# airl-iisc/MRFP

Hardware: AMD Instinct MI355X
Metric: train images/sec (higher is better)
Workload: dtype bf16; 1 GPU; resnet-101 DeepLabV3+ + MRFP+ (HRFP+NP+ on, HRFP re-drawn every step), 768x768, 16 images/GPU, fwd+bwd+SGD, synthetic 19-class, random-init weights; global_batch=16, parallelism=dp1

## Files before the change

### include/mrfp_hip.h

```cpp
#ifndef MRFP_HIP_H
#define MRFP_HIP_H

#include <stdint.h>

#ifdef __cplusplus
extern "C" {
#endif

typedef enum { MRFP_F32 = 0, MRFP_BF16 = 1, MRFP_F16 = 2 } mrfp_dtype;

int mrfp_version(void);
const char* mrfp_last_error(void);

int64_t mrfp_stats_nslab(int64_t B, int64_t Ho);

int mrfp_stats_fwd(const void* x, int dtype, int64_t B, int64_t Ho, int64_t Wo, int64_t C,
                   int64_t Hs, int64_t Ws, const int32_t* tabH, const int32_t* tabW,
                   float* ws, void* stream);

int mrfp_stats_bwd(const void* dy, const void* x, const void* y, const float* mean,
                   const float* fA, const float* fS, int per_image, int dtype, int64_t B, int64_t Ho, int64_t Wo, int64_t C,
                   int64_t Hs, int64_t Ws, const int32_t* tabH, const int32_t* tabW,
                   float* ws, void* stream);
int mrfp_stats_bwd_mask(const void* dy, const void* x, const void* mask, const float* mean, int per_image, int dtype, int64_t B,
// ... 138 lines not shown
                  int64_t sstride, const void* addend, float* colstats, void* stream);
int mrfp_conv_fwd_act(const void* x, const void* wpack, const float* bias, void* y, int dtype,
                      int64_t B, int64_t H, int64_t W, int64_t C, int64_t N, int64_t ldy, int64_t R, int64_t S,
                      int64_t Ho, int64_t Wo, int64_t stride, int64_t pad_h, int64_t pad_w, int64_t dil,
                      int64_t sstride, const void* addend, int act, void* stream);
int mrfp_pack_weight_folded(const float* w, void* wf, const float* conv_bias, const float* bn_weight, const float* bn_bias,
                            const float* running_mean, const float* running_var, float eps, float* bias_out, int dtype,
                            int64_t N, int64_t C, int64_t R, int64_t S, int64_t Npad, int64_t Cpad, void* stream);
int mrfp_pack_weights_folded_batched(const void* jobs, const int64_t* prefix, int64_t njobs, int64_t total, int dtype, void* stream);
int mrfp_conv_stats_layout(int dtype, int64_t B, int64_t H, int64_t W, int64_t C, int64_t N, int64_t ldy, int64_t R, int64_t S,
                           int64_t Ho, int64_t Wo, int64_t stride, int64_t pad_h, int64_t pad_w, int64_t dil, int64_t sstride, int wstats,
                           int64_t* out);
int64_t mrfp_conv_stats_block_rows(int dtype, int64_t B, int64_t H, int64_t W, int64_t C, int64_t N, int64_t R, int64_t S, int64_t Ho,
                                   int64_t Wo, int64_t stride, int64_t pad_h, int64_t pad_w, int64_t dil, int64_t sstride);
int mrfp_conv_single_launch(int64_t B, int64_t image_bytes);
int mrfp_conv_fwd_wstats(const void* x, const void* wpack, const float* bias, void* y, int dtype,
                         int64_t B, int64_t H, int64_t W, int64_t C, int64_t N, int64_t ldy, int64_t R, int64_t S,
                         int64_t Ho, int64_t Wo, int64_t stride, int64_t pad_h, int64_t pad_w, int64_t dil,
                         const uint8_t* rowweight, float* colstats, void* stream);
int mrfp_conv_fwd_gated(const void* x, const void* wpack, const float* bias, void* y, int dtype,
                        int64_t B, int64_t H, int64_t W, int64_t C, int64_t N, int64_t ldy, int64_t R, int64_t S,
                        int64_t Ho, int64_t Wo, int64_t stride, int64_t pad_h, int64_t pad_w, int64_t dil,
                        int64_t sstride, const void* addend, const void* addend_mask, void* stream);
int mrfp_debug_clock_stamps(int family, uint64_t* out, int64_t n);
int64_t mrfp_conv_wgrad_ws_bytes(int64_t M, int64_t N, int64_t Q);
int mrfp_conv_wgrad(const void* x, const void* dy, float* dw, void* ws, int dtype,
                    int64_t B, int64_t H, int64_t W, int64_t C, int64_t Ctrue, int64_t N, int64_t ldn,
                    int64_t R, int64_t S, int64_t Ho, int64_t Wo, int64_t stride, int64_t pad_h, int64_t pad_w,
                    int64_t dil, void* stream);
int64_t mrfp_conv_wgrad_group_max(void);
int64_t mrfp_conv_wgrad_grouped_ws_bytes(int64_t M, int64_t N, int64_t Q, int64_t count);
int mrfp_conv_wgrad_plan(int dtype, int64_t B, int64_t H, int64_t W, int64_t C, int64_t N, int64_t ldn, int64_t R, int64_t S, int64_t Ho,
                         int64_t Wo, int64_t stride, int64_t pad_h, int64_t pad_w, int64_t dil, int64_t count, int64_t* out);
int mrfp_conv_wgrad_grouped(const void* const* xs, const void* const* dys, float* const* dws, int64_t count, void* ws, int dtype,
                            int64_t B, int64_t H, int64_t W, int64_t C, int64_t Ctrue, int64_t N, int64_t ldn,
                            int64_t R, int64_t S, int64_t Ho, int64_t Wo, int64_t stride, int64_t pad_h, int64_t pad_w,
                            int64_t dil, void* stream);
int mrfp_nchw_to_nhwc_pad(const float* x, void* y, int dtype, int64_t B, int64_t C, int64_t H, int64_t W,
                          int64_t Cpad, void* stream);

int mrfp_sgd_step(float* p, const float* g, float* m, int64_t n, float lr, float momentum,
                  float weight_decay, float gscale, int first, void* stream);

int64_t mrfp_grad_check_nblocks(int64_t n);
int mrfp_grad_check(const float* g, int64_t n, float gscale, void* ws, void* state, int dynamic, float growth,
                    float backoff, int growth_interval, float max_norm, void* stream);
// ... 76 lines not shown
```

### mrfp_amd/conv.py

```python
from __future__ import annotations

import collections
import ctypes
import os as _os
import warnings
import weakref
from typing import Any, NamedTuple, Optional

import torch

from . import _lib
from ._lib import call, dt, ptr, stream
from .ops import CL, GRAD_DEFERRED, _chk, channel_sums, empty_cl, grad_sink, notify_grad, wgrad_workspace, zeros_cl
from .ops import _inside_autograd_engine as _in_backward

_PACKS = {}
FUSE_STATS = [_os.environ.get("MRFP_FUSE_STATS", "1") != "0"]


class ConvStats(NamedTuple):
    final: torch.Tensor
    final_count: int
    elements: int
    rows: torch.Tensor
# ... 518 lines not shown
    return t


def _boundary_hook(_grad):
    flush_wgrads()
    return None


GATED_SKIP_HITS = [0]


def ungate(t):
    g = getattr(t, "_mrfp_gate", None) if t is not None else None
    if g is None:
        return t
    if g[1] != t._version:
        raise _lib.MrfpHipError("a gated skip gradient was modified in place before it reached its consumer")
    B, C, H, W = t.shape
    out = empty_cl(B, C, H, W, t.dtype, t.device)
    call("mrfp_affine_bwd_mask", ptr(t), None, ptr(g[0]), ptr(out), None, dt(t), B, H, W, C, None, None, None, 0, stream())
    return out


def L_single(B, H, W, Cphys, Ho, Wo, Nphys, esz):
    return max(B * H * W * Cphys, B * Ho * Wo * Nphys) * esz < 0xF0000000


class _Conv2d(torch.autograd.Function):

    @staticmethod
    def forward(ctx, x, weight, bias, stride, pad_h, pad_w, dil, Nphys, want_skip, stats, wtab):
        B, Cphys, H, W = x.shape
        N, C, R, S = weight.shape
        Ho, Wo = _out_size(H, R, stride, pad_h, dil), _out_size(W, S, stride, pad_w, dil)
        pk = get_pack(weight, bias, x.dtype, Cphys, Nphys)
        y = empty_cl(B, Nphys, Ho, Wo, x.dtype, x.device)
        _lib.NOTE[0] = (C, N)
        if wtab is not None:
            call("mrfp_conv_fwd_wstats", ptr(x), ptr(pk.wf), ptr(pk.bias), ptr(y), dt(x), B, H, W, Cphys, Nphys, Nphys, R, S,
                 Ho, Wo, stride, pad_h, pad_w, dil, ptr(wtab), ptr(stats), stream())
            WSTATS_HITS[0] += 1
        else:
            call("mrfp_conv_fwd", ptr(x), ptr(pk.wf), ptr(pk.bias), ptr(y), dt(x), B, H, W, Cphys, Nphys, Nphys, R, S,
                 Ho, Wo, stride, pad_h, pad_w, dil, 1, None, ptr(stats), stream())
        ctx.save_for_backward(x, weight, bias)
        ctx.cfg = (stride, pad_h, pad_w, dil, Nphys, Ho, Wo)
        ctx.set_materialize_grads(False)
        if want_skip:
            return y, x.view_as(x)
        return y

    @staticmethod
    def backward(ctx, dy, dskip=None):
        x, weight, bias = ctx.saved_tensors
        cell = getattr(ctx, "_mrfp_cell", None)
        if cell is not None and cell[1]:
            g = getattr(dskip, "_mrfp_gate", None) if dskip is not None else None
            if g is None or g[1] != dskip._version:
                raise _lib.MrfpHipError("a gated skip gradient reached its convolution without its gate: the skip alias was "
                                        "also consumed by an operator outside mrfp_amd.ops (set MRFP_GATED_SKIP=0)")
            cell[1] = False
        if dy is None:
            return (ungate(dskip),) + (None,) * 10
        stride, pad_h, pad_w, dil, Nphys, Ho, Wo = ctx.cfg
        dy = _chk(dy, "dy")
        B, Cphys, H, W = x.shape
        N, C, R, S = weight.shape
        dx = dw = db = None
        if ctx.needs_input_grad[0]:
            pk = get_pack(weight, bias, x.dtype, Cphys, Nphys)
            dx = empty_cl(B, Cphys, H, W, x.dtype, x.device)
            gate = None
            if dskip is not None:
                g = getattr(dskip, "_mrfp_gate", None)
                if g is not None:
                    if (g[1] == dskip._version and dskip.dtype == x.dtype and x.element_size() == 2
                            and Cphys % 8 == 0 and dskip.shape == dx.shape and dskip.is_contiguous(memory_format=CL)):
                        gate = g[0]
                    else:
                        dskip = ungate(dskip)
                dskip = _chk(dskip, "dskip")
                if dskip.dtype != x.dtype:
                    dskip = dskip.to(x.dtype)
            _lib.NOTE[0] = (N, C)
            if gate is not None:
                call("mrfp_conv_fwd_gated", ptr(dy), ptr(pk.wd), None, ptr(dx), dt(dy), B, Ho, Wo, Nphys, Cphys, Cphys, R, S, H, W,
                     1, dil * (R - 1) - pad_h, dil * (S - 1) - pad_w, dil, stride, ptr(dskip), ptr(gate), stream())
                GATED_SKIP_HITS[0] += 1
            else:
                call("mrfp_conv_fwd", ptr(dy), ptr(pk.wd), None, ptr(dx), dt(dy), B, Ho, Wo, Nphys, Cphys, Cphys, R, S, H, W,
                     1, dil * (R - 1) - pad_h, dil * (S - 1) - pad_w, dil, stride, ptr(dskip), None, stream())
        if ctx.needs_input_grad[1]:
            sig = (x.dtype, B, H, W, Cphys, C, N, Nphys, R, S, Ho, Wo, stride, pad_h, pad_w, dil)
            sink = grad_sink(weight)
            side = _WGRADS.stream(x.device) if sink is not None else None
            if sink is not None and GROUP_WGRAD[0] and L_single(B, H, W, Cphys, Ho, Wo, Nphys, x.element_size()):
                _WGRADS.submit(sig, x, dy, sink, weight)
            elif side is not None:
                _WGRADS.ensure_callback()
                _launch_wgrads(sig, [(x, dy, sink)], side)
                notify_grad(weight)
            else:
                dw = sink if sink is not None else torch.empty((N, C, R, S), dtype=torch.float32, device=x.device)
                _launch_wgrads(sig, [(x, dy, dw)], None)
                if sink is not None:
                    notify_grad(weight)
                    dw = None
                elif dw.dtype != weight.dtype:
                    dw = dw.to(weight.dtype)
        if bias is not None and ctx.needs_input_grad[2]:
            db = channel_sums(dy, N).to(bias.dtype)
        return (dx, dw, db) + (None,) * 8


class _SharedConv1x1Pair(torch.autograd.Function):

    @staticmethod
    def forward(ctx, x1, x2, weight, bias, Nphys):
        N, C, R, S = weight.shape
        if R != 1 or S != 1 or x1.shape[1] != C or x2.shape[1] != C:
            raise _lib.MrfpHipError("shared conv pair: 1x1 weight and unpadded inputs expected")
        pk = get_pack(weight, bias, x1.dtype, C, Nphys)
        ys = []
        for x, b in ((x1, None), (x2, pk.bias)):
            B, _, H, W = x.shape
            y = empty_cl(B, Nphys, H, W, x.dtype, x.device)
            call("mrfp_conv_fwd", ptr(x), ptr(pk.wf), ptr(b), ptr(y), dt(x), B, H, W, C, Nphys, Nphys, 1, 1, H, W, 1, 0, 0, 1, 1,
                 None, None, stream())
            ys.append(y)
        ctx.save_for_backward(x1, x2, weight, bias)
        ctx.Nphys = Nphys
        ctx.set_materialize_grads(False)
        return ys[0], ys[1]

    @staticmethod
    def backward(ctx, dy1, dy2):
        x1, x2, weight, bias = ctx.saved_tensors
        N, C, _, _ = weight.shape
        Nphys = ctx.Nphys
        pk = get_pack(weight, bias, x1.dtype, C, Nphys)
        dxs, dws = [], []
        db = None
        for x, dy, need_dx in ((x1, dy1, ctx.needs_input_grad[0]), (x2, dy2, ctx.needs_input_grad[1])):
            if dy is None:
                dxs.append(None)
                continue
            dy = _chk(dy, "dy")
            B, _, H, W = x.shape
            dx = None
            if need_dx:
                dx = empty_cl(B, C, H, W, x.dtype, x.device)
                call("mrfp_conv_fwd", ptr(dy), ptr(pk.wd), None, ptr(dx), dt(dy), B, H, W, Nphys, C, C, 1, 1, H, W, 1, 0, 0, 1, 1,
                     None, None, stream())
            dxs.append(dx)
            if ctx.needs_input_grad[2]:
                dw = torch.empty((N, C, 1, 1), dtype=torch.float32, device=x.device)
                _launch_wgrads((x.dtype, B, H, W, C, C, N, Nphys, 1, 1, H, W, 1, 0, 0, 1), [(x, dy, dw)], None)
                dws.append(dw)
        if bias is not None and ctx.needs_input_grad[3] and dy2 is not None:
            db = channel_sums(_chk(dy2, "dy"), N).to(bias.dtype)
        dw = None
        if dws:
            total = dws[0] if len(dws) == 1 else dws[0].add_(dws[1])
            sink = grad_sink(weight)
            if sink is not None:
                sink.copy_(total)
                notify_grad(weight)
            else:
                dw = total.to(weight.dtype)
        return dxs[0], dxs[1], dw, db, None


def shared_conv1x1_pair(x1, x2, weight, bias, phys_out):
# ... 31 lines not shown
                                "path is dense only" % (tuple(weight.shape), x.shape[1], groups))
    Nphys = phys_out if phys_out is not None else _round_up(N, epc)
    B, Cphys, H, W = x.shape
    R, S = weight.shape[2], weight.shape[3]
    Ho, Wo = _out_size(H, R, st, ph, dl), _out_size(W, S, st, pw, dl)
    L = _lib.lib()
    single = bool(L.mrfp_conv_single_launch(B, H * W * Cphys * x.element_size()))
    plan, wtab, stats = stat_resize, None, None
    if plan is not None and WSTATS[0] and FUSE_STATS[0] and single and (plan.Hs, plan.Ws) == (Ho, Wo) and R * S > 1:
        wtab = plan.multiplicity(B)
    if wtab is not None or (bias is None and FUSE_STATS[0] and single):
        lay = (ctypes.c_int64 * 5)()
        rc = L.mrfp_conv_stats_layout(dt(x), B, H, W, Cphys, Nphys, Nphys, R, S, Ho, Wo, st, ph, pw, dl, 1, int(wtab is not None), lay)
        if rc != 0:
            raise _lib.MrfpHipError("mrfp_conv_stats_layout failed (%d): %s" % (rc, L.mrfp_last_error().decode()))
        nblk, rb, rows, first, cnt = lay
        stats = torch.empty(rows * 2 * Nphys, dtype=torch.float32, device=x.device)
    if _WGRADS.callback_queued and not _in_backward():
        _WGRADS.drop_stale()
    out = _Conv2d.apply(x, weight, bias, st, ph, pw, dl, Nphys, want_skip, stats, wtab)
    y, skip = out if want_skip else (out, None)
    if skip is not None:
        skip._mrfp_skip_alias = True
        skip._mrfp_uses = [0, False]
        if y.grad_fn is not None:
            y.grad_fn._mrfp_cell = skip._mrfp_uses
    if stats is not None and (phys_out is not None or Nphys == N):
        final = stats[first * 2 * Nphys:(first + cnt) * 2 * Nphys]
        if wtab is not None:
            y._mrfp_colstats = ConvStats(final, cnt, B * plan.Ho * plan.Wo, stats, nblk, 0, plan, y._version)
        else:
            y._mrfp_colstats = ConvStats(final, cnt, B * Ho * Wo, stats, nblk, rb, None, y._version)
    if phys_out is None and Nphys != N:
        y = y[:, :N].contiguous(memory_format=CL)
    return (y, skip) if want_skip else y
```

### mrfp_amd/csrc/conv_c64.hip

```cpp
#include "conv_common.hpp"

namespace mrfp {


struct C64P {
    const char* x;
    const char* w;
    char* y;
    const float* bias;
    const char* addend;
    float* colstats;
    const unsigned char* rowweight;
    int B, H, W, N, ldy, dil;
    int strips;
    int units;
    int spi;
    unsigned xbytes, wbytes, ybytes;
};

constexpr int kC64Slots = 4;

template <typename T, int CB, int NCG, bool STATS, bool ADD, int ACT = 0>
__global__ __launch_bounds__(256, (CB == 1 ? 2 : 1)) void conv3x3_c64_kernel(C64P p) {
    constexpr int PSN = 4 / NCG;
    constexpr int SW = 64 * PSN;
    constexpr int NPIECE = (SW + 4 + 7) / 8;
    constexpr int NPC = CB * NPIECE;
    constexpr int PWV = (NPC + 3) / 4;
    constexpr int SLOT = NPC * 1024;
    constexpr int KS = 18 * CB;
    constexpr int PIXB = 128 * CB;
    constexpr int ST = 4;
    extern __shared__ __attribute__((aligned(16))) char smem[];
    const int t = threadIdx.x, lane = t & 63;
    const int wave = __builtin_amdgcn_readfirstlane(t >> 6);
    const int l15 = lane & 15, lq = lane >> 4;
    const int cg = wave % NCG, ps = wave / NCG;
    const int n0 = (int)blockIdx.y * 128 + cg * 32, nl = n0 + 8 * lq;
    const int d = p.dil;
    const unsigned lds0 = (unsigned)(size_t)(__attribute__((address_space(3))) char*)smem;
    const i32x4 xw = rsrc_words(p.x, p.xbytes);
    const __amdgpu_buffer_rsrc_t wr = __builtin_amdgcn_make_buffer_rsrc((void*)p.w, 0, (int)p.wbytes, 0x00020000);
    const __amdgpu_buffer_rsrc_t yr = __builtin_amdgcn_make_buffer_rsrc((void*)p.y, 0, (int)p.ybytes, 0x00020000);
    const __amdgpu_buffer_rsrc_t ar = __builtin_amdgcn_make_buffer_rsrc((void*)(p.addend ? p.addend : p.y), 0, (int)p.ybytes, 0x00020000);

    uint4 fw[KS][2];
#pragma unroll
    for (int ks = 0; ks < KS; ++ks)
#pragma unroll
        for (int j = 0; j < 2; ++j) {
            const int n = n0 + 8 * (l15 >> 2) + 4 * j + (l15 & 3);
            fw[ks][j] = bload(wr, n < p.N ? (unsigned)n * (unsigned)(1152 * CB) + (unsigned)(ks * 64 + lq * 16) : kOOB);
        }
#pragma unroll
    for (int ks = 0; ks < KS; ++ks)
#pragma unroll
        for (int j = 0; j < 2; ++j) settle(fw[ks][j]);
    float bv[2][4];
#pragma unroll
    for (int j = 0; j < 2; ++j)
#pragma unroll
        for (int e = 0; e < 4; ++e) bv[j][e] = (p.bias && nl + 4 * j + e < p.N) ? p.bias[nl + 4 * j + e] : 0.f;

    unsigned foff[3][2];
#pragma unroll
    for (int s = 0; s < 3; ++s) {
        const int px = ps * 64 + l15 + s * d;
#pragma unroll
        for (int kk = 0; kk < 2; ++kk) foff[s][kk] = (unsigned)(px * 128 + ((((kk * 4 + lq) ^ px) & 7) << 4));
    }

    float cs[8], cq[8];
#pragma unroll
    for (int u = 0; u < 8; ++u) { cs[u] = 0.f; cq[u] = 0.f; }

    const long long G = gridDim.x;
    int u = (int)((long long)blockIdx.x * p.units / G);
    const int u1 = (int)((long long)(blockIdx.x + 1) * p.units / G);
    const int Hc0 = (p.H + d - 1) / d;
    const int upi = p.strips * p.H;
// ... 62 lines not shown
                const unsigned cb = (unsigned)(col * PIXB + hf * 128 + (((lane & 7) ^ (px & 7)) << 4));
                dma16_async(xw, sbase + (unsigned)(pi * 1024), (rok && cok) ? rbase + cb : kOOB);
            }
        };
        issue_row(i0 - 1);
        issue_row(i0);
        issue_row(i0 + 1);
        for (int i = i0; i < i1; ++i) {
            if (i == i0) dma_wait<0>();
            else dma_wait<ST>();
            __builtin_amdgcn_s_barrier();
            if (i + 1 < i1) issue_row(i + 2);
            const int oh = q + d * i;
            uint4 av[4];
            unsigned wt[4];
            const int owl = ow0 + ps * 64 + l15;
            const unsigned ml = (unsigned)((b * p.H + oh) * p.W + owl);
            auto out_off = [&](int bk) {
                return (owl + bk * 16 < p.W && nl < p.N) ? ((ml + (unsigned)(bk * 16)) * (unsigned)p.ldy + (unsigned)nl) * 2u : kOOB;
            };
#pragma unroll
            for (int bk = 0; bk < 4; ++bk) {
                if constexpr (ADD) av[bk] = bload(ar, out_off(bk));
                if constexpr (STATS) {
                    const bool ok = owl + bk * 16 < p.W;
                    wt[bk] = ok ? (p.rowweight ? (unsigned)p.rowweight[ml + bk * 16] : 1u) : 0u;
                }
            }
            f32x4 acc[4][2];
            const unsigned sb[3] = {lds0 + (unsigned)(((i + 3) & 3) * SLOT), lds0 + (unsigned)((i & 3) * SLOT),
                                    lds0 + (unsigned)(((i + 1) & 3) * SLOT)};
            uint4 fx[2][4];
            auto read_x = [&](int ks, uint4 (&f)[4]) {
                const int r = ks / (6 * CB), s = (ks / (2 * CB)) % 3, hf = (ks >> 1) % CB, kk = ks & 1;
                const char* base = smem + (sb[r] - lds0) + hf * (NPIECE * 1024) + foff[s][kk];
#pragma unroll
                for (int bk = 0; bk < 4; ++bk) f[bk] = *reinterpret_cast<const uint4*>(base + bk * 2048);
            };
            read_x(0, fx[0]);
#pragma unroll
            for (int ks = 0; ks < KS; ++ks) {
                if (ks + 1 < KS) read_x(ks + 1, fx[(ks + 1) & 1]);
                __builtin_amdgcn_sched_barrier(0);
#pragma unroll
                for (int bk = 0; bk < 4; ++bk)
#pragma unroll
                    for (int j = 0; j < 2; ++j) {
                        if (ks == 0) {
                            const f32x4 z = {bv[j][0], bv[j][1], bv[j][2], bv[j][3]};
                            acc[bk][j] = z;
                        }
                        Mma16<T>::run(acc[bk][j], fw[ks][j], fx[ks & 1][bk]);
                    }
                __builtin_amdgcn_sched_barrier(0);
            }
#pragma unroll
            for (int bk = 0; bk < 4; ++bk) {
                uint4 v;
                if constexpr (ADD) {
                    float a[8];
                    unpack2<T>(av[bk].x, a[0], a[1]);
                    unpack2<T>(av[bk].y, a[2], a[3]);
                    unpack2<T>(av[bk].z, a[4], a[5]);
                    unpack2<T>(av[bk].w, a[6], a[7]);
                    v.x = pack2<T>(act_f<ACT>(acc[bk][0][0] + a[0]), act_f<ACT>(acc[bk][0][1] + a[1]));
                    v.y = pack2<T>(act_f<ACT>(acc[bk][0][2] + a[2]), act_f<ACT>(acc[bk][0][3] + a[3]));
                    v.z = pack2<T>(act_f<ACT>(acc[bk][1][0] + a[4]), act_f<ACT>(acc[bk][1][1] + a[5]));
                    v.w = pack2<T>(act_f<ACT>(acc[bk][1][2] + a[6]), act_f<ACT>(acc[bk][1][3] + a[7]));
                } else {
                    v.x = pack2<T>(act_f<ACT>(acc[bk][0][0]), act_f<ACT>(acc[bk][0][1]));
                    v.y = pack2<T>(act_f<ACT>(acc[bk][0][2]), act_f<ACT>(acc[bk][0][3]));
                    v.z = pack2<T>(act_f<ACT>(acc[bk][1][0]), act_f<ACT>(acc[bk][1][1]));
                    v.w = pack2<T>(act_f<ACT>(acc[bk][1][2]), act_f<ACT>(acc[bk][1][3]));
                }
                if constexpr (STATS) {
                    float f[8];
                    unpack2<T>(v.x, f[0], f[1]);
                    unpack2<T>(v.y, f[2], f[3]);
                    unpack2<T>(v.z, f[4], f[5]);
                    unpack2<T>(v.w, f[6], f[7]);
                    const float wb = (float)wt[bk];
#pragma unroll
// ... 29 lines not shown
        if (!c128 || (p.N != 64 && p.N != 128 && p.N != 256)) return false;
        const int SW = p.N == 64 ? 128 : 64;
        if (c128 < 2 && (int64_t)p.B * ((p.W + SW - 1) / SW) * p.H < 32 * kGrid1PerCU) return false;
    } else return false;
    if (p.addend_mask || (p.colstats && p.addend)) return false;
    if ((int64_t)p.M * p.ldy * esz >= (int64_t)kOOB || p.H < 2 * p.dil) return false;
    return true;
}
bool c64_plan(const ConvP& p, int esz, ConvPlan& plan) {
    if (!c64_applicable(p, esz)) return false;
    const int SW = p.N == 64 ? 128 : 64;
    const int64_t upi = (int64_t)((p.W + SW - 1) / SW) * p.H, units = upi * p.B;
    const int64_t cap = p.C == 64 ? kGrid2PerCU : kGrid1PerCU;
    plan.kind = ConvKernel::c64;
    plan.tile_rows = 0;
    plan.grid = (int)(units < cap ? units : cap);
    plan.spi = (int)(upi / (units / plan.grid) + 2);
    const int64_t rows_per_image = (int64_t)(p.N == 64 ? 2 : 1) * plan.spi;
    plan.stats_blocks = p.B * rows_per_image;
    plan.stats_block_rows = -rows_per_image;
    return true;
}

template <typename T, int CB, int NCG, bool STATS, bool ADD, int ACT = 0>
static int c64_launch(const C64P& q, int grid, hipStream_t st) {
    constexpr int SW = 64 * (4 / NCG), NPIECE = (SW + 4 + 7) / 8;
    const int lds = kC64Slots * CB * NPIECE * 1024 + 1024;
    static bool attr_set = false;
    if (!attr_set) {
        (void)hipFuncSetAttribute(reinterpret_cast<const void*>(&conv3x3_c64_kernel<T, CB, NCG, STATS, ADD, ACT>),
                                  hipFuncAttributeMaxDynamicSharedMemorySize, lds);
        attr_set = true;
    }
    hipLaunchKernelGGL((conv3x3_c64_kernel<T, CB, NCG, STATS, ADD, ACT>), dim3((unsigned)grid, (unsigned)((q.N + 127) / 128)), dim3(256), lds, st, q);
    MRFP_LAUNCH_CHECK();
    return 0;
}
template <typename T, int CB, int NCG>
static int c64_pick(const ConvP& p, const C64P& q, int grid, hipStream_t st, int act) {
    if (act != 0) {
        if (p.colstats) return -1;
        if (act == 1) return p.addend ? c64_launch<T, CB, NCG, false, true, 1>(q, grid, st) : c64_launch<T, CB, NCG, false, false, 1>(q, grid, st);
        return p.addend ? c64_launch<T, CB, NCG, false, true, 2>(q, grid, st) : c64_launch<T, CB, NCG, false, false, 2>(q, grid, st);
    }
    if (p.colstats) return c64_launch<T, CB, NCG, true, false>(q, grid, st);
    if (p.addend) return c64_launch<T, CB, NCG, false, true>(q, grid, st);
    return c64_launch<T, CB, NCG, false, false>(q, grid, st);
}

template <typename T>
static int c64_run_t(const ConvP& p, const ConvPlan& plan, hipStream_t st, int act) {
    C64P q;
    q.x = p.x; q.w = p.w; q.y = p.y; q.bias = p.bias; q.addend = p.addend; q.colstats = p.colstats; q.rowweight = p.rowweight;
    q.B = p.B; q.H = p.H; q.W = p.W; q.N = p.N; q.ldy = p.ldy; q.dil = p.dil;
    const int SW = p.N == 64 ? 128 : 64;
    q.strips = (p.W + SW - 1) / SW;
    q.units = p.B * q.strips * p.H;
    q.spi = plan.spi;
    q.xbytes = p.xbytes; q.wbytes = p.wbytes; q.ybytes = (unsigned)((int64_t)p.M * p.ldy * 2);
    const int grid = plan.grid;
    if (p.C == 64) return p.N == 64 ? c64_pick<T, 1, 2>(p, q, grid, st, act) : c64_pick<T, 1, 4>(p, q, grid, st, act);
    return p.N == 64 ? c64_pick<T, 2, 2>(p, q, grid, st, act) : c64_pick<T, 2, 4>(p, q, grid, st, act);
}
int c64_run(const ConvP& p, const ConvPlan& plan, bool is_f16, hipStream_t st, int act) {
    return is_f16 ? c64_run_t<f16>(p, plan, st, act) : c64_run_t<bf16>(p, plan, st, act);
}

}
```

### mrfp_amd/csrc/conv_common.hpp

```cpp
#pragma once
#include "common.hpp"
#include <stdlib.h>

#ifndef MRFP_VMCNT0
#define MRFP_VMCNT0 0
#endif

#ifndef MRFP_CLOCK_STAMP
#define MRFP_CLOCK_STAMP 0
#endif

namespace mrfp {

constexpr int kGrid1PerCU = kCUs;
constexpr int kGrid2PerCU = 2 * kCUs;

constexpr int kStampSlots = 4096;
#if MRFP_CLOCK_STAMP
struct ClockStamp {
    unsigned long long t0, r0;
    __device__ __forceinline__ void begin() {
        t0 = __builtin_amdgcn_s_memtime();
        r0 = __builtin_amdgcn_s_memrealtime();
        __builtin_amdgcn_s_waitcnt(0xC07F);
// ... 219 lines not shown
    return make_uint4(w(v.x, 0), w(v.y, 2), w(v.z, 4), w(v.w, 6));
}

#ifndef MRFP_EARLY_FULL
#define MRFP_EARLY_FULL 1
#endif

enum class ConvKernel { pw, pwk, c64, rr384, rr192, t256x64, t192x128, t96x128, t128x128 };
struct ConvPlan {
    ConvKernel kind;
    int tile_rows;
    int64_t stats_blocks;
    int64_t stats_block_rows;
    int grid, spi;
};

bool pw_plan(const ConvP& p, int esz, ConvPlan& plan);
int pw_run(const ConvP& p, bool is_f16, hipStream_t st, int act = 0);

bool pwk_plan(const ConvP& p, int esz, ConvPlan& plan);
int pwk_run(const ConvP& p, bool is_f16, hipStream_t st, int act = 0);

bool c64_plan(const ConvP& p, int esz, ConvPlan& plan);
int c64_run(const ConvP& p, const ConvPlan& plan, bool is_f16, hipStream_t st, int act = 0);

constexpr int kWgMaxGroup = 32;
struct WgGroup {
    const char* x[kWgMaxGroup];
    const char* dy[kWgMaxGroup];
};
inline WgGroup make_wg_group(const void* const* xs, const void* const* dys, int64_t count) {
    WgGroup g;
    for (int i = 0; i < kWgMaxGroup; ++i) {
        g.x[i] = (const char*)xs[i < count ? i : 0];
        g.dy[i] = (const char*)dys[i < count ? i : 0];
    }
    return g;
}

struct ClassWalk {
    int Wp, a, L, R, Wr, splits;
};
inline bool class_walk(int64_t ncls, int64_t U, int per_round, int64_t count, ClassWalk& w) {
    w.Wp = (int)(per_round / count);
    if (ncls * U < w.Wp) w.Wp = (int)(ncls * U);
    w.a = (int)(w.Wp / ncls);
    if (w.a < 1) return false;
// ... 43 lines not shown
```

### mrfp_amd/csrc/conv_igemm.hip

```cpp
#include "conv_common.hpp"
#include <type_traits>

namespace mrfp {

MRFP_STAMP_DECL(g_stamps_igemm)
int stamps_igemm(unsigned long long* out, int n) { return MRFP_STAMP_READ(g_stamps_igemm, out, n); }

template <typename T, int WM, int WN, bool ALIGNED, bool STRIDED, int TM, int TN, bool RR = false, int ACT = 0>
__global__ __launch_bounds__(64 * WM * WN, ((RR && TM * TN >= 6) ? 2 : 3)) void conv_igemm_kernel(ConvP p) {
    constexpr int NT = 64 * WM * WN, BM = 32 * TM * WM, BN = 32 * TN * WN;
    constexpr int SA = BM * 8 / NT, SB = BN * 8 / NT, RSTEP = NT / 8;
    extern __shared__ __attribute__((aligned(16))) char smem[];
    char* const sA0 = smem;
    char* const sB0 = smem + BM * 128;
    MRFP_STAMP_BEGIN();

    const int t = threadIdx.x, lane = t & 63, wave = t >> 6;
    const int wm = wave / WN, wn = wave % WN;
    const int ntn = (p.N + BN - 1) / BN;
    const int tile = xcd_remap(blockIdx.x, gridDim.x);
    const int m0 = (tile / ntn) * BM, n0 = (tile % ntn) * BN;
    const int rbase = t >> 3;
    const int chunk = (t & 7) ^ ((rbase >> 1) & 7);
    const int wrow = __builtin_amdgcn_readfirstlane(wave) * 8;
// ... 634 lines not shown
    const int esz = dtype_bytes(dtype);
    MRFP_CHECK((C * esz) % 16 == 0, "conv_fwd: C=%lld must make 16-byte chunks (pad the channels)", (long long)C);
    MRFP_CHECK(B * Ho * Wo < (1LL << 31), "conv_fwd: tensor too large for 32-bit tile indices");
    p = ConvP{};
    p.bias = bias; p.addend = (const char*)addend; p.addend_mask = (const unsigned char*)addend_mask;
    p.colstats = colstats; p.rowweight = rowweight;
    p.B = (int)B; p.H = (int)H; p.W = (int)W; p.C = (int)C; p.N = (int)N; p.ldy = (int)ldy;
    p.R = (int)R; p.S = (int)S; p.Ho = (int)Ho; p.Wo = (int)Wo;
    p.stride = (int)stride; p.pad_h = (int)pad_h; p.pad_w = (int)pad_w; p.dil = (int)dil; p.sstride = (int)sstride;
    p.M = (int)(B * Ho * Wo); p.cpr = (int)(C * esz / 16); p.kchunks = (int)(R * S * p.cpr);
    return 0;
}

}

using namespace mrfp;

extern "C" {

static int conv_fwd_impl(const void* x, const void* wpack, const float* bias, void* y, int dtype, int64_t B, int64_t H,
                         int64_t W, int64_t C, int64_t N, int64_t ldy, int64_t R, int64_t S, int64_t Ho, int64_t Wo,
                         int64_t stride, int64_t pad_h, int64_t pad_w, int64_t dil, int64_t sstride, const void* addend,
                         float* colstats, void* stream, const void* addend_mask = nullptr, const unsigned char* rowweight = nullptr,
                         int act = 0) {
    MRFP_CHECK(act >= 0 && act <= 2, "conv_fwd_act: act must be 0 (none), 1 (ReLU) or 2 (ReLU6), got %d", act);
    MRFP_CHECK(act == 0 || (sstride == 1 && !colstats && !addend_mask && !rowweight),
               "conv_fwd_act: an activation is a forward-launch option (sstride 1, no statistics, no gate mask)");
    MRFP_CHECK(!addend || aligned16(addend), "conv_fwd: addend must be 16-byte aligned");
    MRFP_CHECK(!rowweight || (colstats && ((uintptr_t)rowweight & 3) == 0), "conv_fwd_wstats: the row weights need statistics and 4-byte alignment");
    MRFP_CHECK(!addend_mask || (addend && dtype != MRFP_F32 && (N & 7) == 0 && ldy == N),
               "conv_fwd_gated: a gate mask needs an addend, 16-bit activations, N %% 8 == 0 and a dense output");
    MRFP_CHECK(x && wpack && y, "conv_fwd: bad arguments");
    ConvP p;
    const int bad = conv_params(p, dtype, B, H, W, C, N, ldy, R, S, Ho, Wo, stride, pad_h, pad_w, dil, sstride, bias, addend, addend_mask,
                                colstats, rowweight);
    if (bad) return bad;
    MRFP_CHECK(aligned16(x) && aligned16(wpack), "conv_fwd: x / wpack must be 16-byte aligned");
    const int esz = dtype_bytes(dtype);
    p.w = (const char*)wpack;
    ConvPlan plan = conv_plan(p, esz);
    {
        static const int on = env_switch("MRFP_DGRAD_CLASSED", 1);
        p.classed = on && sstride == 2 && stride == 1 && dil == 1 && (Ho & 1) == 0 && (Wo & 1) == 0 && (p.cpr & 7) == 0 &&
                    ((B * (Ho / 2) * (Wo / 2)) % 256) == 0 && !colstats;
        if (p.classed && ((B * (Ho / 2) * (Wo / 2)) % plan.tile_rows) != 0) p.classed = 0;
        if (p.classed && R == 1 && S == 1 && pad_h == 0 && pad_w == 0) p.classed = 2;
    }
    const int64_t img = H * W * C * esz, wb = N * (int64_t)p.kchunks * 16;
    MRFP_CHECK(img < (int64_t)kOOB && wb < (int64_t)kOOB,
               "conv_fwd: one input image / the weight pack exceeds the 3.75 GB buffer-descriptor range");
    const int64_t bmax = (int64_t)(kOOB - 1) / img;
    const bool chunked = B > bmax;
    MRFP_CHECK(!chunked || !colstats, "conv_fwd: fused statistics are not available for inputs above 3.75 GB (see mrfp_conv_single_launch)");
    MRFP_CHECK(!rowweight || plan.kind != ConvKernel::pw, "conv_fwd_wstats: not available on the pointwise kernels");
    if (chunked) p.classed = 0;
    static const int dbg_drop = env_switch("MRFP_DEBUG_DROP", 0);
    int rc = 0;
    for (int64_t b0 = 0; b0 < B && !rc; b0 += bmax) {
        const int64_t bc = B - b0 < bmax ? B - b0 : bmax;
        const int64_t m0 = b0 * Ho * Wo;
        p.B = (int)bc;
        p.M = p.classed == 2 ? (int)(bc * (Ho / 2) * (Wo / 2)) : (int)(bc * Ho * Wo);
        p.x = (const char*)x + b0 * img;
        p.y = (char*)y + m0 * ldy * esz;
        p.addend = addend ? (const char*)addend + m0 * ldy * esz : nullptr;
        p.addend_mask = addend_mask ? (const unsigned char*)addend_mask + ((m0 * ldy) >> 3) : nullptr;
        p.xbytes = (dbg_drop & 1) ? 0u : (unsigned)(bc * img);
        p.wbytes = (dbg_drop & 2) ? 0u : (unsigned)wb;
        if (chunked) plan = conv_plan(p, esz);
        rc = by_dtype(dtype, "conv_fwd", [&](auto t) { return run_igemm_act<typename decltype(t)::type>(p, plan, (hipStream_t)stream, act); });
    }
    if (rc || !colstats) return rc;
    if (plan.stats_blocks > kCompactAbove) {
        const int C2 = 2 * (int)ldy;
        hipLaunchKernelGGL(compact_stats_kernel, dim3((unsigned)((C2 + 63) / 64), kStatGroups), dim3(256), 0,
                           (hipStream_t)stream, colstats, (int)plan.stats_blocks, C2);
        MRFP_LAUNCH_CHECK();
    }
    return 0;
}

int mrfp_debug_clock_stamps(int family, uint64_t* out, int64_t n) {
    MRFP_CHECK(MRFP_CLOCK_STAMP != 0, "clock stamps: not a diagnostic build (-DMRFP_CLOCK_STAMP=1)");
    MRFP_CHECK(out && n > 0 && n <= kStampSlots && family >= 0 && family <= 3, "clock stamps: bad arguments");
    (void)hipDeviceSynchronize();
    const int rc = family == 0 ? stamps_igemm((unsigned long long*)out, (int)n)
                   : family == 1 ? stamps_pw((unsigned long long*)out, (int)n)
                   : family == 2 ? stamps_wgrad((unsigned long long*)out, (int)n) : stamps_pwk((unsigned long long*)out, (int)n);
    MRFP_CHECK(rc == 0, "clock stamps: read-back failed");
    return 0;
}

int mrfp_conv_single_launch(int64_t B, int64_t image_bytes) {
// ... 12 lines not shown
                      int64_t W, int64_t C, int64_t N, int64_t ldy, int64_t R, int64_t S, int64_t Ho, int64_t Wo,
                      int64_t stride, int64_t pad_h, int64_t pad_w, int64_t dil, int64_t sstride, const void* addend,
                      int act, void* stream) {
    return conv_fwd_impl(x, wpack, bias, y, dtype, B, H, W, C, N, ldy, R, S, Ho, Wo, stride, pad_h, pad_w, dil, sstride, addend,
                         nullptr, stream, nullptr, nullptr, act);
}

int mrfp_conv_fwd_wstats(const void* x, const void* wpack, const float* bias, void* y, int dtype, int64_t B, int64_t H,
                         int64_t W, int64_t C, int64_t N, int64_t ldy, int64_t R, int64_t S, int64_t Ho, int64_t Wo,
                         int64_t stride, int64_t pad_h, int64_t pad_w, int64_t dil, const uint8_t* rowweight, float* colstats,
                         void* stream) {
    MRFP_CHECK(rowweight && colstats, "conv_fwd_wstats: row weights and a statistics buffer are required");
    return conv_fwd_impl(x, wpack, bias, y, dtype, B, H, W, C, N, ldy, R, S, Ho, Wo, stride, pad_h, pad_w, dil, 1, nullptr,
                         colstats, stream, nullptr, rowweight);
}

int mrfp_conv_fwd_gated(const void* x, const void* wpack, const float* bias, void* y, int dtype, int64_t B, int64_t H,
                        int64_t W, int64_t C, int64_t N, int64_t ldy, int64_t R, int64_t S, int64_t Ho, int64_t Wo,
                        int64_t stride, int64_t pad_h, int64_t pad_w, int64_t dil, int64_t sstride, const void* addend,
                        const void* addend_mask, void* stream) {
    MRFP_CHECK(addend && addend_mask, "conv_fwd_gated: addend and its gate mask are required");
    return conv_fwd_impl(x, wpack, bias, y, dtype, B, H, W, C, N, ldy, R, S, Ho, Wo, stride, pad_h, pad_w, dil, sstride, addend,
                         nullptr, stream, addend_mask);
}

int mrfp_conv_stats_layout(int dtype, int64_t B, int64_t H, int64_t W, int64_t C, int64_t N, int64_t ldy, int64_t R, int64_t S,
                           int64_t Ho, int64_t Wo, int64_t stride, int64_t pad_h, int64_t pad_w, int64_t dil, int64_t sstride, int wstats,
                           int64_t* out) {
    MRFP_CHECK(out, "conv_stats_layout: no output array");
    float stats_present;
    unsigned char rows_present;
    ConvP p;
    const int bad = conv_params(p, dtype, B, H, W, C, N, ldy, R, S, Ho, Wo, stride, pad_h, pad_w, dil, sstride, nullptr, nullptr,
                                nullptr, &stats_present, wstats ? &rows_present : nullptr);
    if (bad) return bad;
    const ConvPlan plan = conv_plan(p, dtype_bytes(dtype));
    const int64_t nblk = plan.stats_blocks;
    const bool compact = nblk > kCompactAbove;
    out[0] = nblk;
    out[1] = plan.stats_block_rows;
    out[2] = compact ? nblk + kStatGroups : nblk;
    out[3] = compact ? nblk : 0;
    out[4] = compact ? kStatGroups : nblk;
    return 0;
}

// ... 9 lines not shown
```

Before: 307.0 images/sec.

## Fuse low-rank skip gradient into 3x3 dgrad kernel instead of materializing it

Measured after the change: 310.3 images/sec (median of 6 runs). 1.1% higher.

```diff
diff --git a/include/mrfp_hip.h b/include/mrfp_hip.h
--- a/include/mrfp_hip.h
+++ b/include/mrfp_hip.h
@@ -184,6 +184,13 @@
                         int64_t B, int64_t H, int64_t W, int64_t C, int64_t N, int64_t ldy, int64_t R, int64_t S,
                         int64_t Ho, int64_t Wo, int64_t stride, int64_t pad_h, int64_t pad_w, int64_t dil,
                         int64_t sstride, const void* addend, const void* addend_mask, void* stream);
+int mrfp_conv_fwd_lowrank(const void* x, const void* wpack, const float* bias, void* y, int dtype,
+                          int64_t B, int64_t H, int64_t W, int64_t C, int64_t N, int64_t ldy, int64_t R, int64_t S,
+                          int64_t Ho, int64_t Wo, int64_t stride, int64_t pad_h, int64_t pad_w, int64_t dil,
+                          int64_t sstride, const void* addend, float* colstats, const void* lr_x, const void* lr_w, int64_t lr_k,
+                          void* stream);
+int mrfp_conv_lowrank_ok(int dtype, int64_t B, int64_t H, int64_t W, int64_t C, int64_t N, int64_t ldy, int64_t R, int64_t S,
+                         int64_t Ho, int64_t Wo, int64_t stride, int64_t pad_h, int64_t pad_w, int64_t dil);
 int mrfp_debug_clock_stamps(int family, uint64_t* out, int64_t n);
 int64_t mrfp_conv_wgrad_ws_bytes(int64_t M, int64_t N, int64_t Q);
 int mrfp_conv_wgrad(const void* x, const void* dy, float* dw, void* ws, int dtype,
diff --git a/mrfp_amd/conv.py b/mrfp_amd/conv.py
--- a/mrfp_amd/conv.py
+++ b/mrfp_amd/conv.py
@@ -564,6 +564,31 @@
     return out
 
 
+LOWRANK_SKIP = [_os.environ.get("MRFP_LOWRANK_SKIP", "1") != "0"]
+LOWRANK_SKIP_HITS = [0]
+_LOWRANK_K = 32
+
+
+def unlowrank(t):
+    lr = getattr(t, "_mrfp_lowrank", None) if t is not None else None
+    if lr is None:
+        return t
+    dp, wd, K, version = lr
+    if version != t._version:
+        raise _lib.MrfpHipError("a low-rank skip gradient was modified in place before it reached its consumer")
+    B, C, H, W = t.shape
+    out = empty_cl(B, C, H, W, dp.dtype, dp.device)
+    call("mrfp_conv_fwd", ptr(dp), ptr(wd), None, ptr(out), dt(dp), B, H, W, K, C, C, 1, 1, H, W, 1, 0, 0, 1, 1, None, None, stream())
+    return out
+
+
+def _dgrad_lowrank_ok(dtype, B, H, W, Cphys, Nphys, R, S, Ho, Wo, stride, pad_h, pad_w, dil):
+    if dtype not in (torch.bfloat16, torch.float16) or stride != 1:
+        return False
+    return bool(_lib.lib().mrfp_conv_lowrank_ok(_lib._DT[dtype], B, Ho, Wo, Nphys, Cphys, Cphys, R, S, H, W, 1, dil * (R - 1) - pad_h,
+                                                dil * (S - 1) - pad_w, dil))
+
+
 def L_single(B, H, W, Cphys, Ho, Wo, Nphys, esz):
     return max(B * H * W * Cphys, B * Ho * Wo * Nphys) * esz < 0xF0000000
 
@@ -602,8 +627,14 @@
                 raise _lib.MrfpHipError("a gated skip gradient reached its convolution without its gate: the skip alias was "
                                         "also consumed by an operator outside mrfp_amd.ops (set MRFP_GATED_SKIP=0)")
             cell[1] = False
+        lr = getattr(dskip, "_mrfp_lowrank", None) if dskip is not None else None
+        if cell is not None and cell[2]:
+            if lr is None or lr[3] != dskip._version:
+                raise _lib.MrfpHipError("a low-rank skip gradient reached its convolution without its factors: the skip alias was "
+                                        "also consumed by an operator outside mrfp_amd.ops (set MRFP_LOWRANK_SKIP=0)")
+            cell[2] = False
         if dy is None:
-            return (ungate(dskip),) + (None,) * 10
+            return (unlowrank(ungate(dskip)),) + (None,) * 10
         stride, pad_h, pad_w, dil, Nphys, Ho, Wo = ctx.cfg
         dy = _chk(dy, "dy")
         B, Cphys, H, W = x.shape
@@ -613,6 +644,12 @@
             pk = get_pack(weight, bias, x.dtype, Cphys, Nphys)
             dx = empty_cl(B, Cphys, H, W, x.dtype, x.device)
             gate = None
+            if lr is not None:
+                if (lr[3] == dskip._version and lr[2] == _LOWRANK_K and lr[0].dtype == dy.dtype == x.dtype and dskip.shape == dx.shape
+                        and _dgrad_lowrank_ok(x.dtype, B, H, W, Cphys, Nphys, R, S, Ho, Wo, stride, pad_h, pad_w, dil)):
+                    dskip = None
+                else:
+                    dskip, lr = unlowrank(dskip), None
             if dskip is not None:
                 g = getattr(dskip, "_mrfp_gate", None)
                 if g is not None:
@@ -625,7 +662,11 @@
                 if dskip.dtype != x.dtype:
                     dskip = dskip.to(x.dtype)
             _lib.NOTE[0] = (N, C)
-            if gate is not None:
+            if lr is not None:
+                call("mrfp_conv_fwd_lowrank", ptr(dy), ptr(pk.wd), None, ptr(dx), dt(dy), B, Ho, Wo, Nphys, Cphys, Cphys, R, S, H, W,
+                     1, dil * (R - 1) - pad_h, dil * (S - 1) - pad_w, dil, stride, None, None, ptr(lr[0]), ptr(lr[1]), lr[2], stream())
+                LOWRANK_SKIP_HITS[0] += 1
+            elif gate is not None:
                 call("mrfp_conv_fwd_gated", ptr(dy), ptr(pk.wd), None, ptr(dx), dt(dy), B, Ho, Wo, Nphys, Cphys, Cphys, R, S, H, W,
                      1, dil * (R - 1) - pad_h, dil * (S - 1) - pad_w, dil, stride, ptr(dskip), ptr(gate), stream())
                 GATED_SKIP_HITS[0] += 1
@@ -672,6 +713,7 @@
             ys.append(y)
         ctx.save_for_backward(x1, x2, weight, bias)
         ctx.Nphys = Nphys
+        ctx.lr_cell = getattr(x2, "_mrfp_uses", None) if getattr(x2, "_mrfp_lowrank_ok", False) else None
         ctx.set_materialize_grads(False)
         return ys[0], ys[1]
 
@@ -683,14 +725,19 @@
         pk = get_pack(weight, bias, x1.dtype, C, Nphys)
         dxs, dws = [], []
         db = None
-        for x, dy, need_dx in ((x1, dy1, ctx.needs_input_grad[0]), (x2, dy2, ctx.needs_input_grad[1])):
+        for x, dy, need_dx, cell in ((x1, dy1, ctx.needs_input_grad[0], None), (x2, dy2, ctx.needs_input_grad[1], ctx.lr_cell)):
             if dy is None:
                 dxs.append(None)
                 continue
             dy = _chk(dy, "dy")
             B, _, H, W = x.shape
             dx = None
-            if need_dx:
+            if (need_dx and cell is not None and LOWRANK_SKIP[0] and cell[0] == 1 and Nphys == _LOWRANK_K and dy.dtype == x.dtype
+                    and x.element_size() == 2):
+                dx = torch.empty((), dtype=x.dtype, device=x.device).expand(B, C, H, W)
+                dx._mrfp_lowrank = (dy, pk.wd, Nphys, dx._version)
+                cell[2] = True
+            elif need_dx:
                 dx = empty_cl(B, C, H, W, x.dtype, x.device)
                 call("mrfp_conv_fwd", ptr(dy), ptr(pk.wd), None, ptr(dx), dt(dy), B, H, W, Nphys, C, C, 1, 1, H, W, 1, 0, 0, 1, 1,
                      None, None, stream())
@@ -768,7 +815,10 @@
     y, skip = out if want_skip else (out, None)
     if skip is not None:
         skip._mrfp_skip_alias = True
-        skip._mrfp_uses = [0, False]
+        skip._mrfp_uses = [0, False, False]
+        if (LOWRANK_SKIP[0] and y.grad_fn is not None and x.requires_grad
+                and _dgrad_lowrank_ok(x.dtype, B, H, W, Cphys, Nphys, R, S, Ho, Wo, st, ph, pw, dl)):
+            skip._mrfp_lowrank_ok = True
         if y.grad_fn is not None:
             y.grad_fn._mrfp_cell = skip._mrfp_uses
     if stats is not None and (phys_out is not None or Nphys == N):
diff --git a/mrfp_amd/csrc/conv_c64.hip b/mrfp_amd/csrc/conv_c64.hip
--- a/mrfp_amd/csrc/conv_c64.hip
+++ b/mrfp_amd/csrc/conv_c64.hip
@@ -16,12 +16,16 @@
     int units;
     int spi;
     unsigned xbytes, wbytes, ybytes;
+    const char* lr_x;
+    const char* lr_w;
+    unsigned lrbytes;
 };
 
 constexpr int kC64Slots = 4;
 
-template <typename T, int CB, int NCG, bool STATS, bool ADD, int ACT = 0>
+template <typename T, int CB, int NCG, bool STATS, bool ADD, int ACT = 0, bool LR = false>
 __global__ __launch_bounds__(256, (CB == 1 ? 2 : 1)) void conv3x3_c64_kernel(C64P p) {
+    static_assert(!LR || (!STATS && !ADD && ACT == 0), "the low-rank operand excludes statistics, an addend and an activation");
     constexpr int PSN = 4 / NCG;
     constexpr int SW = 64 * PSN;
     constexpr int NPIECE = (SW + 4 + 7) / 8;
@@ -56,6 +60,18 @@
     for (int ks = 0; ks < KS; ++ks)
 #pragma unroll
         for (int j = 0; j < 2; ++j) settle(fw[ks][j]);
+    const __amdgpu_buffer_rsrc_t lxr = __builtin_amdgcn_make_buffer_rsrc((void*)p.lr_x, 0, (int)p.lrbytes, 0x00020000);
+    uint4 fl[2];
+    if constexpr (LR) {
+        const __amdgpu_buffer_rsrc_t lwr = __builtin_amdgcn_make_buffer_rsrc((void*)p.lr_w, 0, p.N * 64, 0x00020000);
+#pragma unroll
+        for (int j = 0; j < 2; ++j) {
+            const int n = n0 + 8 * (l15 >> 2) + 4 * j + (l15 & 3);
+            fl[j] = bload(lwr, n < p.N ? (unsigned)(n * 64 + lq * 16) : kOOB);
+        }
+#pragma unroll
+        for (int j = 0; j < 2; ++j) settle(fl[j]);
+    }
     float bv[2][4];
 #pragma unroll
     for (int j = 0; j < 2; ++j)
@@ -164,6 +180,7 @@
 #pragma unroll
             for (int bk = 0; bk < 4; ++bk) {
                 if constexpr (ADD) av[bk] = bload(ar, out_off(bk));
+                if constexpr (LR) av[bk] = bload(lxr, owl + bk * 16 < p.W ? (ml + (unsigned)(bk * 16)) * 64u + (unsigned)(lq * 16) : kOOB);
                 if constexpr (STATS) {
                     const bool ok = owl + bk * 16 < p.W;
                     wt[bk] = ok ? (p.rowweight ? (unsigned)p.rowweight[ml + bk * 16] : 1u) : 0u;
@@ -196,10 +213,19 @@
                     }
                 __builtin_amdgcn_sched_barrier(0);
             }
+            if constexpr (LR) {
+#pragma unroll
+                for (int bk = 0; bk < 4; ++bk) {
+                    f32x4 t0 = {0.f, 0.f, 0.f, 0.f}, t1 = {0.f, 0.f, 0.f, 0.f};
+                    Mma16<T>::run(t0, fl[0], av[bk]);
+                    Mma16<T>::run(t1, fl[1], av[bk]);
+                    av[bk] = make_uint4(pack2<T>(t0[0], t0[1]), pack2<T>(t0[2], t0[3]), pack2<T>(t1[0], t1[1]), pack2<T>(t1[2], t1[3]));
+                }
+            }
 #pragma unroll
             for (int bk = 0; bk < 4; ++bk) {
                 uint4 v;
-                if constexpr (ADD) {
+                if constexpr (ADD || LR) {
                     float a[8];
                     unpack2<T>(av[bk].x, a[0], a[1]);
                     unpack2<T>(av[bk].y, a[2], a[3]);
@@ -275,22 +301,26 @@
     return true;
 }
 
-template <typename T, int CB, int NCG, bool STATS, bool ADD, int ACT = 0>
+template <typename T, int CB, int NCG, bool STATS, bool ADD, int ACT = 0, bool LR = false>
 static int c64_launch(const C64P& q, int grid, hipStream_t st) {
     constexpr int SW = 64 * (4 / NCG), NPIECE = (SW + 4 + 7) / 8;
     const int lds = kC64Slots * CB * NPIECE * 1024 + 1024;
     static bool attr_set = false;
     if (!attr_set) {
-        (void)hipFuncSetAttribute(reinterpret_cast<const void*>(&conv3x3_c64_kernel<T, CB, NCG, STATS, ADD, ACT>),
+        (void)hipFuncSetAttribute(reinterpret_cast<const void*>(&conv3x3_c64_kernel<T, CB, NCG, STATS, ADD, ACT, LR>),
                                   hipFuncAttributeMaxDynamicSharedMemorySize, lds);
         attr_set = true;
     }
-    hipLaunchKernelGGL((conv3x3_c64_kernel<T, CB, NCG, STATS, ADD, ACT>), dim3((unsigned)grid, (unsigned)((q.N + 127) / 128)), dim3(256), lds, st, q);
+    hipLaunchKernelGGL((conv3x3_c64_kernel<T, CB, NCG, STATS, ADD, ACT, LR>), dim3((unsigned)grid, (unsigned)((q.N + 127) / 128)), dim3(256), lds, st, q);
     MRFP_LAUNCH_CHECK();
     return 0;
 }
 template <typename T, int CB, int NCG>
 static int c64_pick(const ConvP& p, const C64P& q, int grid, hipStream_t st, int act) {
+    if (q.lr_x) {
+        MRFP_CHECK(act == 0 && !p.colstats && !p.addend, "conv_fwd_lowrank: no activation, statistics or addend beside the low-rank operand");
+        return c64_launch<T, CB, NCG, false, false, 0, true>(q, grid, st);
+    }
     if (act != 0) {
         if (p.colstats) return -1;
         if (act == 1) return p.addend ? c64_launch<T, CB, NCG, false, true, 1>(q, grid, st) : c64_launch<T, CB, NCG, false, false, 1>(q, grid, st);
@@ -302,8 +332,9 @@
 }
 
 template <typename T>
-static int c64_run_t(const ConvP& p, const ConvPlan& plan, hipStream_t st, int act) {
+static int c64_run_t(const ConvP& p, const ConvPlan& plan, hipStream_t st, int act, const void* lr_x, const void* lr_w) {
     C64P q;
+    q.lr_x = (const char*)lr_x; q.lr_w = (const char*)lr_w; q.lrbytes = lr_x ? (unsigned)((int64_t)p.M * 64) : 0u;
     q.x = p.x; q.w = p.w; q.y = p.y; q.bias = p.bias; q.addend = p.addend; q.colstats = p.colstats; q.rowweight = p.rowweight;
     q.B = p.B; q.H = p.H; q.W = p.W; q.N = p.N; q.ldy = p.ldy; q.dil = p.dil;
     const int SW = p.N == 64 ? 128 : 64;
@@ -315,8 +346,9 @@
     if (p.C == 64) return p.N == 64 ? c64_pick<T, 1, 2>(p, q, grid, st, act) : c64_pick<T, 1, 4>(p, q, grid, st, act);
     return p.N == 64 ? c64_pick<T, 2, 2>(p, q, grid, st, act) : c64_pick<T, 2, 4>(p, q, grid, st, act);
 }
-int c64_run(const ConvP& p, const ConvPlan& plan, bool is_f16, hipStream_t st, int act) {
-    return is_f16 ? c64_run_t<f16>(p, plan, st, act) : c64_run_t<bf16>(p, plan, st, act);
-}
-
-}
+int c64_run(const ConvP& p, const ConvPlan& plan, bool is_f16, hipStream_t st, int act, const void* lr_x, const void* lr_w) {
+    MRFP_CHECK(!lr_x == !lr_w, "conv_fwd_lowrank: both low-rank operands or neither");
+    return is_f16 ? c64_run_t<f16>(p, plan, st, act, lr_x, lr_w) : c64_run_t<bf16>(p, plan, st, act, lr_x, lr_w);
+}
+
+}
diff --git a/mrfp_amd/csrc/conv_common.hpp b/mrfp_amd/csrc/conv_common.hpp
--- a/mrfp_amd/csrc/conv_common.hpp
+++ b/mrfp_amd/csrc/conv_common.hpp
@@ -265,7 +265,8 @@
 int pwk_run(const ConvP& p, bool is_f16, hipStream_t st, int act = 0);
 
 bool c64_plan(const ConvP& p, int esz, ConvPlan& plan);
-int c64_run(const ConvP& p, const ConvPlan& plan, bool is_f16, hipStream_t st, int act = 0);
+int c64_run(const ConvP& p, const ConvPlan& plan, bool is_f16, hipStream_t st, int act = 0, const void* lr_x = nullptr,
+            const void* lr_w = nullptr);
 
 constexpr int kWgMaxGroup = 32;
 struct WgGroup {
diff --git a/mrfp_amd/csrc/conv_igemm.hip b/mrfp_amd/csrc/conv_igemm.hip
--- a/mrfp_amd/csrc/conv_igemm.hip
+++ b/mrfp_amd/csrc/conv_igemm.hip
@@ -680,7 +680,7 @@
                          int64_t W, int64_t C, int64_t N, int64_t ldy, int64_t R, int64_t S, int64_t Ho, int64_t Wo,
                          int64_t stride, int64_t pad_h, int64_t pad_w, int64_t dil, int64_t sstride, const void* addend,
                          float* colstats, void* stream, const void* addend_mask = nullptr, const unsigned char* rowweight = nullptr,
-                         int act = 0) {
+                         int act = 0, const void* lr_x = nullptr, const void* lr_w = nullptr) {
     MRFP_CHECK(act >= 0 && act <= 2, "conv_fwd_act: act must be 0 (none), 1 (ReLU) or 2 (ReLU6), got %d", act);
     MRFP_CHECK(act == 0 || (sstride == 1 && !colstats && !addend_mask && !rowweight),
                "conv_fwd_act: an activation is a forward-launch option (sstride 1, no statistics, no gate mask)");
@@ -712,6 +712,8 @@
     MRFP_CHECK(!chunked || !colstats, "conv_fwd: fused statistics are not available for inputs above 3.75 GB (see mrfp_conv_single_launch)");
     MRFP_CHECK(!rowweight || plan.kind != ConvKernel::pw, "conv_fwd_wstats: not available on the pointwise kernels");
     if (chunked) p.classed = 0;
+    MRFP_CHECK(!lr_x || (plan.kind == ConvKernel::c64 && !chunked),
+               "conv_fwd_lowrank: these operands do not run on the weight-stationary 3x3 kernel (see mrfp_conv_lowrank_ok)");
     static const int dbg_drop = env_switch("MRFP_DEBUG_DROP", 0);
     int rc = 0;
     for (int64_t b0 = 0; b0 < B && !rc; b0 += bmax) {
@@ -726,7 +728,8 @@
         p.xbytes = (dbg_drop & 1) ? 0u : (unsigned)(bc * img);
         p.wbytes = (dbg_drop & 2) ? 0u : (unsigned)wb;
         if (chunked) plan = conv_plan(p, esz);
-        rc = by_dtype(dtype, "conv_fwd", [&](auto t) { return run_igemm_act<typename decltype(t)::type>(p, plan, (hipStream_t)stream, act); });
+        if (lr_x) rc = c64_run(p, plan, dtype == MRFP_F16, (hipStream_t)stream, 0, lr_x, lr_w);
+        else rc = by_dtype(dtype, "conv_fwd", [&](auto t) { return run_igemm_act<typename decltype(t)::type>(p, plan, (hipStream_t)stream, act); });
     }
     if (rc || !colstats) return rc;
     if (plan.stats_blocks > kCompactAbove) {
@@ -785,6 +788,28 @@
     MRFP_CHECK(addend && addend_mask, "conv_fwd_gated: addend and its gate mask are required");
     return conv_fwd_impl(x, wpack, bias, y, dtype, B, H, W, C, N, ldy, R, S, Ho, Wo, stride, pad_h, pad_w, dil, sstride, addend,
                          nullptr, stream, addend_mask);
+}
+
+int mrfp_conv_fwd_lowrank(const void* x, const void* wpack, const float* bias, void* y, int dtype, int64_t B, int64_t H,
+                          int64_t W, int64_t C, int64_t N, int64_t ldy, int64_t R, int64_t S, int64_t Ho, int64_t Wo,
+                          int64_t stride, int64_t pad_h, int64_t pad_w, int64_t dil, int64_t sstride, const void* addend,
+                          float* colstats, const void* lr_x, const void* lr_w, int64_t lr_k, void* stream) {
+    MRFP_CHECK(!addend && !colstats, "conv_fwd_lowrank: the low-rank operand excludes an addend and statistics");
+    MRFP_CHECK(lr_x && lr_w && aligned16(lr_x) && aligned16(lr_w), "conv_fwd_lowrank: both low-rank operands are required, 16-byte aligned");
+    MRFP_CHECK(lr_k == 32, "conv_fwd_lowrank: the low-rank K is 32, got %lld", (long long)lr_k);
+    MRFP_CHECK(dtype == MRFP_BF16 || dtype == MRFP_F16, "conv_fwd_lowrank: 16-bit activations only (dtype %d)", dtype);
+    return conv_fwd_impl(x, wpack, bias, y, dtype, B, H, W, C, N, ldy, R, S, Ho, Wo, stride, pad_h, pad_w, dil, sstride, nullptr,
+                         nullptr, stream, nullptr, nullptr, 0, lr_x, lr_w);
+}
+
+int mrfp_conv_lowrank_ok(int dtype, int64_t B, int64_t H, int64_t W, int64_t C, int64_t N, int64_t ldy, int64_t R, int64_t S,
+                         int64_t Ho, int64_t Wo, int64_t stride, int64_t pad_h, int64_t pad_w, int64_t dil) {
+    if (!dtype_known(dtype) || dtype_bytes(dtype) != 2) return 0;
+    ConvP p;
+    if (conv_params(p, dtype, B, H, W, C, N, ldy, R, S, Ho, Wo, stride, pad_h, pad_w, dil, 1, nullptr, nullptr, nullptr, nullptr, nullptr))
+        return 0;
+    if (!mrfp_conv_single_launch(B, H * W * C * 2)) return 0;
+    return conv_plan(p, 2).kind == ConvKernel::c64 ? 1 : 0;
 }
 
 int mrfp_conv_stats_layout(int dtype, int64_t B, int64_t H, int64_t W, int64_t C, int64_t N, int64_t ldy, int64_t R, int64_t S,
```
